# DrorT/demucs

Measured on AMD Instinct MI355X. Metric: real-time factor (audio-sec/wall-sec) htdemucs 4-stem 44.1kHz stereo, 1/8 GPU, higher is better.
Workload: dtype f32

## Files before the change

demucs_amd/csrc/attention_x6.hip:

```cpp
#include "common.h"
#include "kernels.h"
#include "split_bf16.h"

namespace mi {

namespace {

typedef float f32x16 __attribute__((ext_vector_type(16)));
typedef unsigned u32x4 __attribute__((ext_vector_type(4)));
constexpr int HD = 64;
constexpr int KT = 64;

__device__ __forceinline__ f32x16 mfma6(const u32x4 (&a)[3], const u32x4 (&b)[3], f32x16 acc) {
    constexpr int PA[6] = {2, 0, 1, 1, 0, 0}, PB[6] = {0, 2, 1, 0, 1, 0};
#pragma unroll
    for (int q = 0; q < 6; ++q)
        acc = __builtin_amdgcn_mfma_f32_32x32x16_bf16(__builtin_bit_cast(bf16x8, a[PA[q]]), __builtin_bit_cast(bf16x8, b[PB[q]]), acc, 0,
                                                      0, 0);
    return acc;
}

__device__ __forceinline__ void split8(const float (&x)[8], u32x4 (&out)[3]) {
    unsigned h[4], m[4], l[4];
#pragma unroll
    for (int j = 0; j < 4; ++j) split3(x[2 * j], x[2 * j + 1], h[j], m[j], l[j]);
    out[0] = u32x4{h[0], h[1], h[2], h[3]};
    out[1] = u32x4{m[0], m[1], m[2], m[3]};
    out[2] = u32x4{l[0], l[1], l[2], l[3]};
}

}

__global__ __launch_bounds__(256, 2) void attention_x6_kernel(const float *__restrict__ q, const float *__restrict__ k,
                                                              const float *__restrict__ v, float *__restrict__ o, int Tq, int Tk,
                                                              int64_t q_bs, int64_t kv_bs, int64_t o_bs, int planes, int heads) {
    __shared__ u32x4 Kx[3 * 8 * KT];
    __shared__ u32x4 Vx[3 * 8 * HD];
    {
        float agpr_anchor = 0.f;
        asm volatile("; accumulators in AGPRs %0" : "+a"(agpr_anchor));
    }
    const int tid = threadIdx.x, lane = tid & 63;
    const int wave = __builtin_amdgcn_readfirstlane(tid >> 6);
    const int li = lane & 31, lh = lane >> 5;
    const int nqb = (Tq + 127) / 128;
    const int xj = blockIdx.x >> 3;
    const int pl = (xj / nqb) * 8 + (blockIdx.x & 7);
    if (pl >= planes) return;
    const int head = pl % heads, b = pl / heads;
    const int q0 = (xj % nqb) * 128 + wave * 32;
    const float *qp = q + (size_t)b * q_bs + (size_t)head * HD * Tq;
    const float *kp = k + (size_t)b * kv_bs + (size_t)head * HD * Tk;
    const float *vp = v + (size_t)b * kv_bs + (size_t)head * HD * Tk;

    const int qi = q0 + li;
    const bool qok = qi < Tq;
    const int qic = qok ? qi : Tq - 1;
    u32x4 qx[4][3];
#pragma unroll
    for (int t = 0; t < 4; ++t) {
        float x[8];
#pragma unroll
        for (int j = 0; j < 8; ++j) {
            const float qv = qp[(size_t)(16 * t + 8 * lh + j) * Tq + qic];
            x[j] = qok ? qv * 0.125f : 0.f;
        }
        split8(x, qx[t]);
    }

    f32x16 oacc[2];
#pragma unroll
    for (int r = 0; r < 16; ++r) { oacc[0][r] = 0.f; oacc[1][r] = 0.f; }
    float mrun = -INFINITY, lrun = 0.f;

    const int ve = lane >> 3, vd = (lane & 7) + 8 * wave, vc = 16 * (ve >> 1) + 4 * (ve & 1);
    float kst[2][8];
    float4 vst[2][2];
    auto stage_load = [&](int k0) {
        const bool kok = k0 + lane < Tk;
        const int kc = kok ? k0 + lane : Tk - 1;
#pragma unroll
        for (int i = 0; i < 2; ++i)
#pragma unroll
            for (int j = 0; j < 8; ++j) kst[i][j] = kp[(size_t)(8 * (wave + 4 * i) + j) * Tk + kc];
#pragma unroll
        for (int i = 0; i < 2; ++i)
#pragma unroll
            for (int c = 0; c < 2; ++c) {
                const int key = k0 + vc + 8 * c;
                vst[i][c] = *reinterpret_cast<const float4 *>(vp + (size_t)(vd + 32 * i) * Tk + (key < Tk ? key : Tk - 4));
            }
    };
    auto stage_mask = [&](int k0) {
        if (k0 + KT <= Tk) return;
        if (k0 + lane >= Tk) {
#pragma unroll
            for (int i = 0; i < 2; ++i)
#pragma unroll
                for (int j = 0; j < 8; ++j) kst[i][j] = 0.f;
        }
#pragma unroll
        for (int c = 0; c < 2; ++c)
            if (k0 + vc + 8 * c >= Tk)
#pragma unroll
                for (int i = 0; i < 2; ++i) vst[i][c] = make_float4(0.f, 0.f, 0.f, 0.f);
    };
    auto stage_store = [&]() {
#pragma unroll
        for (int i = 0; i < 2; ++i) {
            u32x4 t[3];
            split8(kst[i], t);
#pragma unroll
            for (int p = 0; p < 3; ++p) Kx[(p * 8 + wave + 4 * i) * KT + lane] = t[p];
        }
#pragma unroll
        for (int i = 0; i < 2; ++i) {
            const float x[8] = {vst[i][0].x, vst[i][0].y, vst[i][0].z, vst[i][0].w, vst[i][1].x, vst[i][1].y, vst[i][1].z, vst[i][1].w};
            u32x4 t[3];
            split8(x, t);
#pragma unroll
            for (int p = 0; p < 3; ++p) Vx[(p * 8 + ve) * HD + vd + 32 * i] = t[p];
        }
    };

    stage_load(0);
    for (int k0 = 0; k0 < Tk; k0 += KT) {
        __syncthreads();
        stage_mask(k0);
        stage_store();
        __syncthreads();
        if (k0 + KT < Tk) stage_load(k0 + KT);
#pragma unroll
        for (int sub = 0; sub < 2; ++sub) {
            const int kb = sub * 32;
            if (k0 + kb >= Tk) break;
            f32x16 sacc;
#pragma unroll
            for (int r = 0; r < 16; ++r) sacc[r] = 0.f;
#pragma unroll
            for (int t = 0; t < 4; ++t) {
                u32x4 kf[3];
#pragma unroll
                for (int p = 0; p < 3; ++p) kf[p] = Kx[(p * 8 + 2 * t + lh) * KT + kb + li];
                sacc = mfma6(kf, qx[t], sacc);
            }
            float s[16];
#pragma unroll
            for (int r = 0; r < 16; ++r) s[r] = sacc[r];
            float mloc = -INFINITY;
            if (k0 + kb + 32 > Tk) {
#pragma unroll
                for (int r = 0; r < 16; ++r)
                    if (k0 + kb + (r & 3) + 8 * (r >> 2) + 4 * lh >= Tk) s[r] = -INFINITY;
            }
#pragma unroll
            for (int r = 0; r < 16; ++r) mloc = fmaxf(mloc, s[r]);
            mloc = fmaxf(mloc, __shfl_xor(mloc, 32));
            const float mnew = fmaxf(mrun, mloc);
            float psum = 0.f;
#pragma unroll
            for (int r = 0; r < 16; ++r) {
                const float p = __expf(s[r] - mnew);
                s[r] = p;
                psum += p;
            }
            if (__any(mnew != mrun)) {
                const float alpha = __expf(mrun - mnew);
                lrun *= alpha;
#pragma unroll
                for (int r = 0; r < 16; ++r) { oacc[0][r] *= alpha; oacc[1][r] *= alpha; }
                mrun = mnew;
            }
            lrun += psum;
#pragma unroll
            for (int m = 0; m < 2; ++m) {
                float x[8];
#pragma unroll
                for (int j = 0; j < 8; ++j) x[j] = s[8 * m + j];
                u32x4 px[3];
                split8(x, px);
#pragma unroll
                for (int dt = 0; dt < 2; ++dt) {
                    u32x4 vf[3];
#pragma unroll
                    for (int p = 0; p < 3; ++p) vf[p] = Vx[(p * 8 + 2 * (2 * sub + m) + lh) * HD + dt * 32 + li];
                    oacc[dt] = mfma6(vf, px, oacc[dt]);
                }
            }
        }
    }
    const float ltot = lrun + __shfl_xor(lrun, 32);
    const float inv = 1.0f / ltot;
    if (qok) {
        float *op = o + (size_t)b * o_bs + (size_t)head * HD * Tq + qi;
#pragma unroll
        for (int dt = 0; dt < 2; ++dt)
#pragma unroll
            for (int r = 0; r < 16; ++r) {
                const int dd = dt * 32 + (r & 3) + 8 * (r >> 2) + 4 * lh;
                op[(size_t)dd * Tq] = oacc[dt][r] * inv;
            }
    }
}

int launch_attention_x6(const float *q, const float *k, const float *v, float *o, int B, int heads, int Tq, int Tk, int64_t q_bs,
                        int64_t kv_bs, int64_t o_bs, hipStream_t st) {
    MI_REQUIRE(Tk % 4 == 0, "attention x6: Tk %% 4 != 0 (%d)", Tk);
    MI_REQUIRE(((uintptr_t)k & 15) == 0 && ((uintptr_t)v & 15) == 0 && kv_bs % 4 == 0, "attention x6: k/v must be 16-byte aligned");
    const int planes = B * heads;
    hipLaunchKernelGGL(attention_x6_kernel, dim3((unsigned)(ceil_div(Tq, 128) * ((planes + 7) / 8) * 8)), dim3(256), 0, st, q, k, v, o,
                       Tq, Tk, q_bs, kv_bs, o_bs, planes, heads);
    MI_CHECK_LAUNCH();
    return MI_OK;
}

}
```

Measured before the change: 2361.

## Use lazy softmax rescaling with exp2 and scalar-base 32-bit staging offsets

Replaces per-tile online-softmax max tracking with a lazy reference max that rescales the accumulators only when a new max exceeds the reference by a threshold (TAU=8). Exponentials are computed with exp2 and a fused multiply-add instead of expf of a difference. K/V global loads now use per-row base pointers held in scalar registers plus 32-bit byte offsets, which cuts 64-bit address arithmetic. Empty asm constraints pin the accumulators in AGPRs and keep the Q fragments in VGPRs. The gain in exchange is fewer rescale passes and cheaper exponentials and addressing. The cost is unnormalized probabilities up to e^8, a new requirement that Tk stay below 2^24, and a register allocation that is more tightly constrained.

```diff
diff --git a/demucs_amd/csrc/attention_x6.hip b/demucs_amd/csrc/attention_x6.hip
--- a/demucs_amd/csrc/attention_x6.hip
+++ b/demucs_amd/csrc/attention_x6.hip
@@ -8,8 +8,12 @@
 
 typedef float f32x16 __attribute__((ext_vector_type(16)));
 typedef unsigned u32x4 __attribute__((ext_vector_type(4)));
+typedef __attribute__((address_space(1))) char gchar;
+typedef __attribute__((address_space(1))) float gfloat;
 constexpr int HD = 64;
 constexpr int KT = 64;
+constexpr float LOG2E = 1.44269504088896340736f;
+constexpr float TAU = 8.0f;
 
 __device__ __forceinline__ f32x16 mfma6(const u32x4 (&a)[3], const u32x4 (&b)[3], f32x16 acc) {
     constexpr int PA[6] = {2, 0, 1, 1, 0, 0}, PB[6] = {0, 2, 1, 0, 1, 0};
@@ -71,24 +75,33 @@
     f32x16 oacc[2];
 #pragma unroll
     for (int r = 0; r < 16; ++r) { oacc[0][r] = 0.f; oacc[1][r] = 0.f; }
-    float mrun = -INFINITY, lrun = 0.f;
+    float mref = -INFINITY, nml2 = INFINITY, lrun = 0.f;
 
     const int ve = lane >> 3, vd = (lane & 7) + 8 * wave, vc = 16 * (ve >> 1) + 4 * (ve & 1);
     float kst[2][8];
     float4 vst[2][2];
+    const gchar *krow[2][8];
+#pragma unroll
+    for (int i = 0; i < 2; ++i)
+#pragma unroll
+        for (int j = 0; j < 8; ++j) {
+            krow[i][j] = (const gchar *)(kp + (size_t)(8 * (wave + 4 * i) + j) * Tk);
+            asm("" : "+s"(krow[i][j]));
+        }
     auto stage_load = [&](int k0) {
         const bool kok = k0 + lane < Tk;
-        const int kc = kok ? k0 + lane : Tk - 1;
+        const unsigned kc = 4u * (unsigned)(kok ? k0 + lane : Tk - 1);
 #pragma unroll
         for (int i = 0; i < 2; ++i)
 #pragma unroll
-            for (int j = 0; j < 8; ++j) kst[i][j] = kp[(size_t)(8 * (wave + 4 * i) + j) * Tk + kc];
+            for (int j = 0; j < 8; ++j) kst[i][j] = *(const gfloat *)(krow[i][j] + kc);
 #pragma unroll
         for (int i = 0; i < 2; ++i)
 #pragma unroll
             for (int c = 0; c < 2; ++c) {
                 const int key = k0 + vc + 8 * c;
-                vst[i][c] = *reinterpret_cast<const float4 *>(vp + (size_t)(vd + 32 * i) * Tk + (key < Tk ? key : Tk - 4));
+                const unsigned vo = 4u * ((unsigned)((lane & 7) * Tk) + (unsigned)(key < Tk ? key : Tk - 4));
+                vst[i][c] = *reinterpret_cast<const float4 *>(reinterpret_cast<const char *>(vp + (size_t)(8 * wave + 32 * i) * Tk) + vo);
             }
     };
     auto stage_mask = [&](int k0) {
@@ -125,6 +138,7 @@
 
     stage_load(0);
     for (int k0 = 0; k0 < Tk; k0 += KT) {
+        asm volatile("" : "+a"(oacc[0]), "+a"(oacc[1]));
         __syncthreads();
         stage_mask(k0);
         stage_store();
@@ -134,6 +148,9 @@
         for (int sub = 0; sub < 2; ++sub) {
             const int kb = sub * 32;
             if (k0 + kb >= Tk) break;
+            asm volatile("" : "+a"(oacc[0]), "+a"(oacc[1]));
+#pragma unroll
+            for (int t = 0; t < 4; ++t) asm volatile("" : "+v"(qx[t][0]), "+v"(qx[t][1]), "+v"(qx[t][2]));
             f32x16 sacc;
 #pragma unroll
             for (int r = 0; r < 16; ++r) sacc[r] = 0.f;
@@ -156,20 +173,27 @@
 #pragma unroll
             for (int r = 0; r < 16; ++r) mloc = fmaxf(mloc, s[r]);
             mloc = fmaxf(mloc, __shfl_xor(mloc, 32));
-            const float mnew = fmaxf(mrun, mloc);
+            if (k0 + kb == 0) {
+                mref = mloc;
+                nml2 = -(mloc * LOG2E);
+            }
+            if (__any(mloc > mref + TAU)) {
+                const bool up = mloc > mref + TAU;
+                const float nnew = -(mloc * LOG2E);
+                const float alpha = up ? __builtin_amdgcn_exp2f(nnew - nml2) : 1.0f;
+                mref = up ? mloc : mref;
+                nml2 = up ? nnew : nml2;
+                lrun *= alpha;
+#pragma unroll
+                for (int r = 0; r < 16; ++r) { oacc[0][r] *= alpha; oacc[1][r] *= alpha; }
+            }
+            asm volatile("" : "+a"(oacc[0]), "+a"(oacc[1]));
             float psum = 0.f;
 #pragma unroll
             for (int r = 0; r < 16; ++r) {
-                const float p = __expf(s[r] - mnew);
+                const float p = __builtin_amdgcn_exp2f(__builtin_fmaf(s[r], LOG2E, nml2));
                 s[r] = p;
                 psum += p;
-            }
-            if (__any(mnew != mrun)) {
-                const float alpha = __expf(mrun - mnew);
-                lrun *= alpha;
-#pragma unroll
-                for (int r = 0; r < 16; ++r) { oacc[0][r] *= alpha; oacc[1][r] *= alpha; }
-                mrun = mnew;
             }
             lrun += psum;
 #pragma unroll
@@ -206,6 +230,7 @@
 int launch_attention_x6(const float *q, const float *k, const float *v, float *o, int B, int heads, int Tq, int Tk, int64_t q_bs,
                         int64_t kv_bs, int64_t o_bs, hipStream_t st) {
     MI_REQUIRE(Tk % 4 == 0, "attention x6: Tk %% 4 != 0 (%d)", Tk);
+    MI_REQUIRE(Tk < (1 << 24), "attention x6: Tk %d too long for 32-bit staging offsets", Tk);
     MI_REQUIRE(((uintptr_t)k & 15) == 0 && ((uintptr_t)v & 15) == 0 && kv_bs % 4 == 0, "attention x6: k/v must be 16-byte aligned");
     const int planes = B * heads;
     hipLaunchKernelGGL(attention_x6_kernel, dim3((unsigned)(ceil_div(Tq, 128) * ((planes + 7) / 8) * 8)), dim3(256), 0, st, q, k, v, o,
```

After: 2408 (median of 6 runs). +2.0%, better.
